# codeslake/RefVSR

Hardware: AMD Instinct MI355X
Metric: 4x SR frames/sec (270p->1080p, RefVSR_small_L1) (higher is better)
Workload: dtype f16; 1 GPU; config_RefVSR_small_L1 4x SR, 270x480 -> 1080x1920, frame_num=5, steady-state sliding window, n=1 (BASELINE configs[1]); synthetic clip seed 0, seeded random weights 1234; frames_per_rank=20, parallelism=frame-shard x1 (reset-aligned, no collective), window_cache=True, frame_ids=True, pipelined_calls=True, frames_per_call=4, headline_mode=frame groups, pipe_layout=pfm, full=False

## Files before the change

### include/refvsr_hip.h

```cpp
#ifndef REFVSR_HIP_H
#define REFVSR_HIP_H

#include <stddef.h>
#include <stdint.h>

#ifdef __cplusplus
extern "C" {
#endif

#define REFVSR_ABI_VERSION 15

int refvsr_abi_version(void);
int refvsr_max_maps(void);
const char* refvsr_last_error(void);
int refvsr_init(void);

int refvsr_num_cus(void);
int refvsr_stream_create_cu_range(int first_cu, int n_cus, void** stream);
int refvsr_stream_set_cu_budget(void* stream, int n_cus);
int refvsr_stream_destroy(void* stream);

enum { REFVSR_OUT_NHWC16 = 0, REFVSR_OUT_NHWC16_SHUFFLE2 = 1, REFVSR_OUT_PLANAR32 = 2 };

typedef struct RefvsrConv {
    const void* src0; int c0;
    const void* src1; int c1;
    int h_in, w_in;
    int h_out, w_out;
    int ksize, stride, pad;
    const void* wpack;
    const float* bias;
    int cout;
    int mt_per_block;
    int ksteps;
    float act_slope;
    const void* mul; int mul_c;
    const void* res; int res_c;
    float post_slope;
    int out_mode;
    void* out; int out_c;
    const float* res_planar;
    int f32;
    float add_const;
    float clamp_lo, clamp_hi;
    int batch; size_t bs_src0, bs_src1, bs_out, bs_res_planar;
} RefvsrConv;

int refvsr_conv_mfma(const RefvsrConv* d, void* stream);
int refvsr_set_conv_workgroup_cap(int cap);
int refvsr_conv_variant(const RefvsrConv* d, int* key);
int refvsr_kslot(int ty, int tx, int cg, int ksize, int ncg);
int refvsr_ksteps(int ksize, int ncg);

int refvsr_resblock_lean_fits(int c);
int refvsr_resblock_chain(const void* src, int c, int h, int w, int n, const void* const* w1, const float* const* b1,
                          const void* const* w2, const float* const* b2, int ksteps, float act_slope, float post_slope,
                          void* scratch0, void* scratch1, void* out, void* stream);
int refvsr_set_resblock_waves(int waves);
int refvsr_resblock_lean(const void* src, int c, int h, int w, const void* w1, const float* b1,
                         const void* w2, const float* b2, int ksteps, float act_slope, float post_slope,
                         void* out, void* stream);
#define REFVSR_RESBLOCK24_BLOB_BYTES 43264
int refvsr_resblock24_chain(const void* src, int h, int w, int n, const void* blobs, size_t blob_stride, float act_slope,
                            void* scratch0, void* scratch1, void* out, void* stream);
#define REFVSR_MAX_MAPS 4
int refvsr_resblock24_chain_batch(const void* const* src, int batch, int h, int w, int n, const void* blobs, size_t blob_stride,
                                  float act_slope, void* scratch0, void* scratch1, void* const* out, void* stream);
int refvsr_resblock24_kblock(int s, int q);
#define REFVSR_RESBLOCK24_F16W_BLOB_BYTES 28928
int refvsr_resblock24_f16w_blob_bytes(void);
int refvsr_resblock24_chain_f16w(const void* src, int h, int w, int n, const void* blobs, size_t blob_stride, float act_slope,
                                 void* scratch0, void* scratch1, void* out, void* stream);
int refvsr_resblock24_chain_batch_f16w(const void* const* src, int batch, int h, int w, int n, const void* blobs, size_t blob_stride,
                                       float act_slope, void* scratch0, void* scratch1, void* const* out, void* stream);
int refvsr_set_resblock24_waves(int waves);
#define REFVSR_RESBLOCK48_BLOB_BYTES 172544
int refvsr_resblock48_chain(const void* src, int h, int w, int n, const void* blobs, size_t blob_stride, float act_slope,
                            void* scratch0, void* scratch1, void* out, void* stream);
int refvsr_resblock48_chain_batch(const void* const* src, int batch, int h, int w, int n, const void* blobs, size_t blob_stride,
                                  float act_slope, void* scratch0, void* scratch1, void* const* out, void* stream);
int refvsr_set_resblock24_store(int mode);
int refvsr_conv24_supported(int c0, int c1);
int refvsr_conv24_blob_bytes(int c0, int c1);
int refvsr_conv24_kblock(int ncg, int s, int q);
int refvsr_conv24(const void* src0, int c0, const void* src1, int c1, int h, int w, const void* blob, float act_slope,
                  const void* mul, const void* res, float post_slope, void* out, void* stream);
int refvsr_conv24_batch(const void* const* src0, int c0, const void* const* src1, int c1, int batch, int h, int w, const void* blob,
                        float act_slope, const void* const* mul, const void* const* res, float post_slope, void* const* out,
                        void* stream);
int refvsr_conv_last_supported(int c);
int refvsr_conv_last_blob_bytes(int c);
int refvsr_conv_last(const void* src, int c, int h, int w, const void* blob, const float* base_lr, int bh, int bw,
                     float* out, void* stream);
int refvsr_conv_hr_last(const void* src, int h, int w, const void* blob, float act_slope, const float* base_lr, int bh, int bw,
                        float* out, void* stream);
enum { REFVSR_RESULT_F32 = 0, REFVSR_RESULT_F16 = 1, REFVSR_RESULT_U8 = 2 };
#define REFVSR_RESULT_FMT_MASK 0x0f
#define REFVSR_RESULT_HWC 0x10
int refvsr_convert_result_hwc(const float* src, int h, int w, int out_fmt, void* out, void* stream);
int refvsr_conv_last_fmt(const void* src, int c, int h, int w, const void* blob, const float* base_lr, int bh, int bw,
                         void* out, int out_fmt, void* stream);
int refvsr_conv_hr_last_fmt(const void* src, int h, int w, const void* blob, float act_slope, const float* base_lr, int bh, int bw,
                            void* out, int out_fmt, void* stream);
// ... 151 lines not shown
```

### refvsr_amd/csrc/conv_mfma.hip

```cpp
#include <type_traits>

#include "common.h"
#include "conv_plan.h"

struct ConvArgs {
    const unsigned char* src0; const unsigned char* src1;
    int c0, c1, ncg0, ncg, ps;
    int pixb0, pixb1;
    int h_in, w_in, h_out, w_out;
    int ks, stride, pad;
    int LH, LW;
    int G, S;
    float inv_ncg;
    const uint4* wpack; const float* bias;
    int cout;
    float act_slope, post_slope;
    const unsigned char* mul; int mul_c;
    const unsigned char* res; int res_c;
    int out_mode; void* out; int out_c;
    const float* res_planar; float add_const, clamp_lo, clamp_hi;
    int tab_bytes, wl_bytes;
    int gather;
    int tiles_x, n_xy;
    int prefetch;
    int grid;
    int ring;
    int batch;
    unsigned long long bs_src0, bs_src1, bs_out, bs_res_planar;
};

template <int MT, int TILES, bool F32, bool GATHER, bool RESIDENT, int EPI = 0, int NW = 4, bool HI1 = false>
__global__ __launch_bounds__(NW * 64) __attribute__((amdgpu_waves_per_eu(2, 4))) void conv_mfma_kernel(ConvArgs p) {
    constexpr int NT = NW * 64;
    static_assert(!(GATHER && RESIDENT), "gather mode streams its weights");
    static_assert(EPI == 0 || (RESIDENT && !F32), "the lean epilogue is built for the resident fp16 kernels");
    static_assert(!HI1 || (!F32 && !RESIDENT && !GATHER), "single-fp16 weights are built for the streamed fp16 kernels");
    constexpr int WFR = (F32 || HI1) ? 1 : 2;
    extern __shared__ __attribute__((aligned(16))) unsigned char smem[];
    int* tab = reinterpret_cast<int*>(smem);
    unsigned char* wl = smem + p.tab_bytes;
    unsigned char* tile = wl + p.wl_bytes;

    asm volatile("" :: "s"(p.src0), "s"(p.src1), "s"(p.wpack), "s"(p.bias), "s"(p.out), "s"(p.mul), "s"(p.res), "s"(p.c0),
                 "s"(p.ncg0), "s"(p.ncg), "s"(p.ps), "s"(p.pixb0), "s"(p.pixb1), "s"(p.h_in), "s"(p.w_in), "s"(p.h_out),
                 "s"(p.w_out), "s"(p.ks), "s"(p.stride), "s"(p.pad), "s"(p.LH), "s"(p.LW), "s"(p.G), "s"(p.S), "s"(p.inv_ncg),
                 "s"(p.cout), "s"(p.tab_bytes), "s"(p.wl_bytes), "s"(p.tiles_x), "s"(p.n_xy), "s"(p.grid));
    if (p.batch > 1) {
        const unsigned long long bi = blockIdx.y;
        p.src0 += bi * p.bs_src0;
        if (p.src1) p.src1 += bi * p.bs_src1;
        p.out = reinterpret_cast<unsigned char*>(p.out) + bi * p.bs_out;
        if (p.res_planar) p.res_planar = reinterpret_cast<const float*>(reinterpret_cast<const unsigned char*>(p.res_planar) + bi * p.bs_res_planar);
    }
    const int tid = threadIdx.x;
    const int lane = tid & 63;
    const int wave = tid >> 6;
    const int q = lane >> 4;
    const int lr = lane & 15;
    const int lp = (p.stride == 1) ? rv_pix16(lr) : lr;
    constexpr int TH = NW * TILES / 2;
    const int zg = blockIdx.z;

    for (int g = tid; g < p.S * 4; g += NT) {
        int off, slot;
        if (g < p.G) {
            const int tap = (int)(((float)g + 0.5f) * p.inv_ncg);
            const int cg = g - tap * p.ncg;
            const int ty = tap / p.ks;
            const int tx = tap - ty * p.ks;
            off = GATHER ? (ty | (tx << 8) | (cg << 16)) : ((ty * p.LW + tx) * p.ps + cg) * 16;
            slot = rv_kslot(ty, tx, cg, p.ks, p.ncg);
        } else {
            const int j = g - p.G;
            slot = rv_kpad_slot(j, p.ks, p.ncg);
            off = GATHER ? -1 : (slot < p.G ? 0 : (p.ncg > 1 ? 16 : (p.ks > 1 ? p.ps * 16 : 0)));
        }
        tab[slot] = off;
    }

    int pbase[TILES];
    if constexpr (!GATHER) {
#pragma unroll
        for (int t = 0; t < TILES; ++t) {
            const int ti = wave * TILES + t;
            pbase[t] = (((ti >> 1) * p.stride) * p.LW + ((ti & 1) * 16 + lp) * p.stride) * p.ps * 16;
// ... 288 lines not shown
                asm volatile("" : "+v"(e));
                if (e >= 0)
                    *reinterpret_cast<uint4*>(tile + (((e & 31) * p.LW + ((e >> 5) & 127)) * p.ps + ((e >> 20) & 127)) * 16) = xv[k];
            }
        };
        if (tl < k_hi) { x_fetch(tl); x_park(); }
        __syncthreads();
        for (; tl < k_hi; tl += k_step) {
            const bool has_next = tl + k_step < k_hi;
            if (has_next && p.prefetch) x_fetch(tl + k_step);
            asm volatile("" ::: "memory");
            zero_acc();
            compute_steps(wl, 0, p.S);
            __syncthreads();
            if (has_next) {
                if (!p.prefetch) x_fetch(tl + k_step);
                x_park();
            }
            asm volatile("" ::: "memory");
            int tide = tid;
            asm volatile("" : "+v"(tide));
            const int tyi = tl / p.tiles_x;
            if constexpr (EPI == 1) epilogue_lean(tyi * TH, (tl - tyi * p.tiles_x) * CONV_TW, tide);
            else epilogue(tyi * TH, (tl - tyi * p.tiles_x) * CONV_TW, tide);
            __syncthreads();
        }
    } else {
        const int tl = blockIdx.x;
        const int tyi = tl / p.tiles_x;
        const int tx0 = (tl - tyi * p.tiles_x) * CONV_TW;
        const int ty0 = tyi * TH;
        constexpr int PPW = GATHER ? 1 : CONV_CH * MT * WFR / NW;
        static_assert(GATHER || (PPW * NW == CONV_CH * MT * WFR && PPW >= 1 && 2 * PPW <= 60), "pieces per wave and chunk");
        constexpr int SLOT = CONV_CH * MT * WFR * 1024;
        const int NS = p.ring;
        const int wv = __builtin_amdgcn_readfirstlane(wave);
        const unsigned char* gw = reinterpret_cast<const unsigned char*>(wsrc) + lane * 16;
        auto issue = [&](const int c, const int slot) {
            const int np = min(CONV_CH, p.S - c * CONV_CH) * MT * WFR;
            const unsigned char* g = gw + (size_t)c * SLOT;
            unsigned char* l = wl + slot * SLOT;
#pragma unroll
            for (int j = 0; j < PPW; ++j) {
                const int pc = wv + j * NW;
                __builtin_amdgcn_global_load_lds((const __attribute__((address_space(1))) void*)(g + min(pc, np - 1) * 1024),
                                                 (__attribute__((address_space(3))) void*)(l + pc * 1024), 16, 0, 0);
            }
        };
        int slot_w = 0;
        if constexpr (!GATHER) {
            const int n_chunks = (p.S + CONV_CH - 1) / CONV_CH;
            for (int c = 0; c < min(NS - 1, n_chunks); ++c) { issue(c, slot_w); slot_w = slot_w + 1 == NS ? 0 : slot_w + 1; }
        }
        if constexpr (!GATHER) {
            const int iy0 = ty0 * p.stride - p.pad;
            const int ix0 = tx0 * p.stride - p.pad;
            const int row_chunks = p.LW * p.ncg;
            const float inv_rc = 1.0f / (float)row_chunks;
            const int total = p.LH * row_chunks;
            constexpr int SB = 8;
            for (int idx0 = tid; idx0 < total; idx0 += SB * NT) {
                uint4 sv[SB];
                int sd[SB];
#pragma unroll
                for (int k = 0; k < SB; ++k) {
                    const int idx = min(idx0 + k * NT, total - 1);
                    const int r = (int)(((float)idx + 0.5f) * inv_rc);
                    const int i = idx - r * row_chunks;
                    const int c = (int)(((float)i + 0.5f) * p.inv_ncg);
                    const int cg = i - c * p.ncg;
                    const int iy = iy0 + r;
                    const int ix = ix0 + c;
                    const bool ok = (unsigned)iy < (unsigned)p.h_in && (unsigned)ix < (unsigned)p.w_in;
                    const size_t pix = (size_t)min(max(iy, 0), p.h_in - 1) * p.w_in + min(max(ix, 0), p.w_in - 1);
                    const unsigned char* g = (cg < p.ncg0) ? p.src0 + pix * p.pixb0 + cg * 16 : p.src1 + pix * p.pixb1 + (cg - p.ncg0) * 16;
                    uint4 v = *reinterpret_cast<const uint4*>(g);
                    const unsigned keep = ok ? 0xffffffffu : 0u;
                    v.x &= keep; v.y &= keep; v.z &= keep; v.w &= keep;
                    sv[k] = v;
                    sd[k] = ((r * p.LW + c) * p.ps + cg) * 16;
                }
#pragma unroll
                for (int k = 0; k < SB; ++k)
                    if (idx0 + k * NT < total) *reinterpret_cast<uint4*>(tile + sd[k]) = sv[k];
            }
        } else {
#pragma unroll
            for (int t = 0; t < TILES; ++t) {
                const int ti = wave * TILES + t;
                const int iy = (ty0 + (ti >> 1)) * p.stride - p.pad + 4096, ix = (tx0 + (ti & 1) * 16 + lp) * p.stride - p.pad + 4096;
                pbase[t] = (iy << 16) | ix;
            }
        }
        if constexpr (!GATHER) {
            const unsigned lds_tab = (unsigned)(size_t)(__attribute__((address_space(3))) unsigned char*)reinterpret_cast<unsigned char*>(tab);
            const unsigned lds_wl = (unsigned)(size_t)(__attribute__((address_space(3))) unsigned char*)wl;
            const unsigned lds_tile = (unsigned)(size_t)(__attribute__((address_space(3))) unsigned char*)tile;
            unsigned pbaddr[TILES];
#pragma unroll
            for (int t = 0; t < TILES; ++t) pbaddr[t] = lds_tile + (unsigned)pbase[t];
            typedef unsigned u32x4 __attribute__((ext_vector_type(4)));
            auto ld128 = [](const unsigned addr) {
                u32x4 v;
                asm volatile("ds_read_b128 %0, %1" : "=v"(v) : "v"(addr));
                return make_uint4(v[0], v[1], v[2], v[3]);
            };
            auto tie = [](uint4& r) {
                u32x4 t = {r.x, r.y, r.z, r.w};
                asm volatile("" : "+v"(t));
                r = make_uint4(t[0], t[1], t[2], t[3]);
            };
            auto wait_set = [&](uint4 (&a)[NA], uint4 (&b)[TILES]) {
                asm volatile("s_waitcnt lgkmcnt(%0)" :: "n"(NA + TILES) : "memory");
#pragma unroll
                for (int i = 0; i < NA; ++i) tie(a[i]);
#pragma unroll
                for (int t = 0; t < TILES; ++t) tie(b[t]);
            };
            static_assert(NA + TILES <= 15, "lgkmcnt range");
            auto compute_chunk = [&](const unsigned wslot, const int s0, const int ns) {
                unsigned toff[CONV_CH];
#pragma unroll
                for (int j = 0; j < CONV_CH; ++j)
                    asm volatile("ds_read_b32 %0, %1" : "=v"(toff[j]) : "v"(lds_tab + (unsigned)(((s0 + min(j, ns - 1)) * 4 + q) * 4)));
                asm volatile("s_waitcnt lgkmcnt(0)" ::: "memory");
#pragma unroll
                for (int j = 0; j < CONV_CH; ++j) asm volatile("" : "+v"(toff[j]));
                const unsigned wa = wslot + (unsigned)lane * 16;
                auto load_set = [&](auto jc, uint4 (&a)[NA], uint4 (&b)[TILES]) {
                    constexpr int j = decltype(jc)::value;
                    const unsigned wj = wa + (unsigned)min(j, ns - 1) * (NA * 1024);
#pragma unroll
                    for (int i = 0; i < NA; ++i) {
                        u32x4 v;
                        asm volatile("ds_read_b128 %0, %1 offset:%2" : "=v"(v) : "v"(wj), "n"(i * 1024));
                        a[i] = make_uint4(v[0], v[1], v[2], v[3]);
                    }
#pragma unroll
                    for (int t = 0; t < TILES; ++t) b[t] = ld128(pbaddr[t] + toff[j]);
                };
                uint4 a0[NA], b0[TILES], a1[NA], b1[TILES];
                load_set(std::integral_constant<int, 0>{}, a0, b0);
#define RV_RING_PAIR(J)                                                                     \
                load_set(std::integral_constant<int, (J) + 1>{}, a1, b1);                   \
                wait_set(a0, b0);                                                           \
                __builtin_amdgcn_sched_barrier(0);                                          \
                if ((J) < ns) mfma_step(a0, b0);                                            \
                load_set(std::integral_constant<int, (J) + 2>{}, a0, b0);                   \
                wait_set(a1, b1);                                                           \
                __builtin_amdgcn_sched_barrier(0);                                          \
                if ((J) + 1 < ns) mfma_step(a1, b1);
                RV_RING_PAIR(0) RV_RING_PAIR(2) RV_RING_PAIR(4)
#undef RV_RING_PAIR
                static_assert(CONV_CH == 8, "the ring loop is unrolled for 8 K-steps per chunk");
                load_set(std::integral_constant<int, 7>{}, a1, b1);
                wait_set(a0, b0);
                __builtin_amdgcn_sched_barrier(0);
                if (6 < ns) mfma_step(a0, b0);
                asm volatile("s_waitcnt lgkmcnt(0)" ::: "memory");
#pragma unroll
                for (int i = 0; i < NA; ++i) tie(a1[i]);
#pragma unroll
                for (int t = 0; t < TILES; ++t) tie(b1[t]);
                __builtin_amdgcn_sched_barrier(0);
                if (7 < ns) mfma_step(a1, b1);
            };
            const int n_chunks = (p.S + CONV_CH - 1) / CONV_CH;
            zero_acc();
            int slot_r = 0;
            for (int c = 0; c < n_chunks; ++c) {
                const int after = min(NS - 2, n_chunks - 1 - c);
                if (after <= 0) asm volatile("s_waitcnt vmcnt(0)" ::: "memory");
                else if (after == 1) asm volatile("s_waitcnt vmcnt(%0)" :: "n"(PPW) : "memory");
                else asm volatile("s_waitcnt vmcnt(%0)" :: "n"(2 * PPW) : "memory");
                asm volatile("s_waitcnt lgkmcnt(0)" ::: "memory");
                __builtin_amdgcn_s_barrier();
                asm volatile("" ::: "memory");
                if (c + NS - 1 < n_chunks) { issue(c + NS - 1, slot_w); slot_w = slot_w + 1 == NS ? 0 : slot_w + 1; }
                compute_chunk(lds_wl + (unsigned)slot_r * SLOT, c * CONV_CH, min(CONV_CH, p.S - c * CONV_CH));
                slot_r = slot_r + 1 == NS ? 0 : slot_r + 1;
            }
        } else {
            constexpr int WPT = (CONV_CH * MT * WFR * 64) / NT;
            const int n_chunks = (p.S + CONV_CH - 1) / CONV_CH;
            static_assert(WPT <= 12, "prefetch register set");
            uint4 w0, w1, w2, w3, w4, w5, w6, w7, w8, w9, w10, w11;
    #define RV_W_ALL(OP) OP(0) OP(1) OP(2) OP(3) OP(4) OP(5) OP(6) OP(7) OP(8) OP(9) OP(10) OP(11)
    #define RV_W_LOAD(k) if constexpr (WPT > k) w##k = g[min(tid + k * NT, n16n - 1)];
    #define RV_W_STORE(k) if constexpr (WPT > k) { if (tid + k * NT < n16n) d[tid + k * NT] = w##k; }
            {
                const int n16 = min(CONV_CH, p.S) * MT * WFR * 64;
                uint4* d = reinterpret_cast<uint4*>(wl);
                for (int i = tid; i < n16; i += NT) d[i] = wsrc[i];
            }
            zero_acc();
            __syncthreads();
            for (int c = 0; c < n_chunks; ++c) {
                const int s0 = c * CONV_CH;
                const int ns = min(CONV_CH, p.S - s0);
                const bool has_next = (c + 1 < n_chunks);
                const int sn = has_next ? s0 + CONV_CH : s0;
                const int n16n = min(CONV_CH, p.S - sn) * MT * WFR * 64;
                {
                    const uint4* g = wsrc + (size_t)sn * MT * WFR * 64;
                    RV_W_ALL(RV_W_LOAD)
                }
                compute_steps(wl, s0, ns);
                if (has_next) {
                    __syncthreads();
                    uint4* d = reinterpret_cast<uint4*>(wl);
                    RV_W_ALL(RV_W_STORE)
                    __syncthreads();
                }
            }
        }
        epilogue(ty0, tx0, tid);
    }
}

static int g_wg_cap = 0;
extern "C" int refvsr_set_conv_workgroup_cap(int cap) {
    g_wg_cap = cap > 0 ? cap : 0;
    return 0;
}

extern "C" int refvsr_kslot(int ty, int tx, int cg, int ksize, int ncg) { return rv_kslot(ty, tx, cg, ksize, ncg); }
extern "C" int refvsr_ksteps(int ksize, int ncg) { return rv_ksteps(ksize, ncg); }

template <int MT, int TILES, bool F32, bool GATHER, bool RESIDENT, int EPI, int NW, bool HI1>
static int launch_conv(ConvArgs& a, int nz, size_t lds, hipStream_t st) {
    static RvLaunchCap lc = {};
    int gx = a.n_xy, cap = 0;
    if (int rc = rv_launch_cap(lc, &conv_mfma_kernel<MT, TILES, F32, GATHER, RESIDENT, EPI, NW, HI1>, NW * 64, 160 * 1024, lds, st,
                               RESIDENT ? &cap : nullptr, nz * a.batch))
        return rc;
    if (RESIDENT) {
        if (g_wg_cap > 0) cap = g_wg_cap;
        if (gx > cap) gx = cap;
    }
    a.grid = gx;
    hipLaunchKernelGGL((conv_mfma_kernel<MT, TILES, F32, GATHER, RESIDENT, EPI, NW, HI1>), dim3(gx, a.batch, nz), dim3(NW * 64), lds, st, a);
    RV_LAUNCH_CHECK();
    return 0;
}

static ConvArgs conv_args(const RefvsrConv* d, const ConvPlan& p) {
    const int cgrp = p.F32 ? 4 : 8, esz = p.F32 ? 4 : 2;
    ConvArgs a;
    memset(&a, 0, sizeof(a));
    a.src0 = (const unsigned char*)d->src0; a.src1 = (const unsigned char*)d->src1;
    a.c0 = d->c0; a.c1 = d->c1;
    a.pixb0 = d->c0 * esz; a.pixb1 = d->c1 * esz;
    a.ncg0 = d->c0 / cgrp; a.ncg = (d->c0 + d->c1) / cgrp;
    a.ps = p.ps;
    a.h_in = d->h_in; a.w_in = d->w_in; a.h_out = d->h_out; a.w_out = d->w_out;
    a.ks = d->ksize; a.stride = d->stride; a.pad = d->pad;
    a.LH = p.LH; a.LW = p.LW;
    a.G = p.G; a.S = p.S;
    a.inv_ncg = 1.0f / (float)a.ncg;
    a.wpack = (const uint4*)d->wpack; a.bias = d->bias; a.cout = d->cout;
    a.act_slope = d->act_slope; a.post_slope = d->post_slope;
    a.mul = (const unsigned char*)d->mul; a.mul_c = d->mul_c;
    a.res = (const unsigned char*)d->res; a.res_c = d->res_c;
    a.out_mode = d->out_mode; a.out = d->out; a.out_c = d->out_c;
    a.res_planar = d->res_planar; a.add_const = d->add_const;
    a.clamp_lo = d->clamp_lo; a.clamp_hi = d->clamp_hi;
    a.tab_bytes = p.tab_bytes; a.wl_bytes = p.wl_bytes;
    a.gather = p.gather; a.ring = p.ring; a.prefetch = p.prefetch;
    a.tiles_x = p.tiles_x; a.n_xy = p.n_xy;
    a.batch = d->batch > 1 ? d->batch : 1;
    if (a.batch > 1) { a.bs_src0 = d->bs_src0; a.bs_src1 = d->bs_src1; a.bs_out = d->bs_out; a.bs_res_planar = d->bs_res_planar; }
    return a;
}

static const ConvKnobs& conv_knobs() {
    static const ConvKnobs knobs = conv_knobs_from_env();
    return knobs;
}

extern "C" int refvsr_conv_variant(const RefvsrConv* d, int* key) {
    RV_CHECK(key != nullptr, "conv_variant: null key");
    ConvPlan p;
    if (int rc = conv_plan(d, conv_knobs(), &p)) return rc;
    *key = p.key();
    return 0;
}

extern "C" int refvsr_conv_mfma(const RefvsrConv* d, void* stream) {
    ConvPlan p;
    if (int rc = conv_plan(d, conv_knobs(), &p)) return rc;
    RV_CHECK(refvsr_init() == 0, "init failed");
    ConvArgs a = conv_args(d, p);
    switch (p.key()) {
#define RV_CONV_CASE(...) case conv_variant_key(__VA_ARGS__): return launch_conv<__VA_ARGS__>(a, p.nz, p.lds, (hipStream_t)stream);
        RV_CONV_VARIANTS(RV_CONV_CASE)
#undef RV_CONV_CASE
    }
    refvsr_set_error("conv: no kernel for MT=%d tiles=%d", p.MT, p.TILES);
    return 1;
}
```

### refvsr_amd/csrc/conv_plan.h

```cpp
#pragma once
#include <stddef.h>
#include <stdlib.h>

#include "../../include/refvsr_hip.h"
#include "plan_common.h"

#define CONV_CH 8
#define CONV_RES_MAX 16
#define CONV_XPF 8
#define CONV_TW 32

#define RV_CONV_VARIANTS(X)                                                                                          \
                                                                          \
    X(1, 4, false, true, false, 0, 4, false) X(2, 4, false, true, false, 0, 4, false) X(3, 4, false, true, false, 0, 4, false) \
                                                       \
    X(1, 2, false, false, false, 0, 8, true) X(2, 2, false, false, false, 0, 8, true)                                \
    X(1, 4, false, false, false, 0, 4, true) X(2, 4, false, false, false, 0, 4, true)                                \
    X(1, 2, false, false, false, 0, 4, true) X(2, 2, false, false, false, 0, 4, true)                                \
                                                                               \
    X(3, 2, false, false, true, 1, 16, false) X(3, 2, false, false, true, 0, 16, false)                              \
    X(2, 2, false, false, true, 1, 16, false) X(2, 2, false, false, true, 0, 16, false)                              \
                                                               \
    X(1, 2, false, false, true, 1, 8, false) X(1, 2, false, false, true, 0, 8, false) X(1, 2, false, false, false, 0, 8, false) \
    X(2, 2, false, false, true, 1, 8, false) X(2, 2, false, false, true, 0, 8, false) X(2, 2, false, false, false, 0, 8, false) \
    X(3, 2, false, false, true, 1, 8, false) X(3, 2, false, false, true, 0, 8, false) X(3, 2, false, false, false, 0, 8, false) \
                                                                                     \
    X(1, 1, true, false, true, 0, 8, false) X(1, 1, true, false, false, 0, 8, false)                                 \
    X(2, 1, true, false, true, 0, 8, false) X(2, 1, true, false, false, 0, 8, false)                                 \
               \
    RV_CONV_VARIANTS4(X, 1, 2) RV_CONV_VARIANTS4(X, 1, 4) RV_CONV_VARIANTS4(X, 2, 2) RV_CONV_VARIANTS4(X, 2, 4)     \
    RV_CONV_VARIANTS4(X, 3, 2) RV_CONV_VARIANTS4(X, 3, 4)
#define RV_CONV_VARIANTS4(X, M, T)                                                                                   \
    X(M, T, true, false, true, 0, 4, false) X(M, T, true, false, false, 0, 4, false)                                 \
    X(M, T, false, false, true, 1, 4, false) X(M, T, false, false, true, 0, 4, false) X(M, T, false, false, false, 0, 4, false)

constexpr int conv_variant_key(int MT, int TILES, bool F32, bool GATHER, bool RESIDENT, int EPI, int NW, bool HI1) {
    return MT | TILES << 2 | NW << 6 | EPI << 11 | (int)F32 << 12 | (int)GATHER << 13 | (int)RESIDENT << 14 | (int)HI1 << 15;
}

struct ConvKnobs {
    bool no_persist = false;
    int res_max = CONV_RES_MAX;
    int tiles = 0;
    bool no_w16 = false;
    int ring = 0;
    bool no_nw8 = false;
    bool no_prefetch = false;
    bool no_lean_epi = false;
};
static inline ConvKnobs conv_knobs_from_env() {
    ConvKnobs k;
    auto num = [](const char* name, int dflt) { const char* v = getenv(name); return v ? atoi(v) : dflt; };
    k.no_persist = getenv("REFVSR_CONV_NO_PERSIST") != nullptr;
    k.res_max = num("REFVSR_CONV_RES_MAX", CONV_RES_MAX);
    k.tiles = num("REFVSR_CONV_TILES", 0);
    k.no_w16 = getenv("REFVSR_CONV_NO_W16") != nullptr;
    k.ring = num("REFVSR_CONV_RING", 0);
    k.no_nw8 = getenv("REFVSR_CONV_NO_NW8") != nullptr;
    k.no_prefetch = getenv("REFVSR_CONV_NO_PREFETCH") != nullptr;
    k.no_lean_epi = getenv("REFVSR_CONV_NO_LEAN_EPI") != nullptr;
    return k;
}

struct ConvPlan {
    int MT, TILES; bool F32, GATHER, RESIDENT; int EPI, NW; bool HI1;
    int nz;
    size_t lds;
    int tab_bytes, wl_bytes;
    int ring;
    int LH, LW;
    int ps;
    int G, S;
    int tiles_x, n_xy;
    int gather;
    int prefetch;
    int key() const { return conv_variant_key(MT, TILES, F32, GATHER, RESIDENT, EPI, NW, HI1); }
};

static int conv_plan(const RefvsrConv* d, const ConvKnobs& knobs, ConvPlan* p) {
    RV_CHECK(d != nullptr, "conv: null descriptor");
    *p = ConvPlan();
    const bool f32 = d->f32 == 1;
    const bool hi1 = d->f32 == 2;
    RV_CHECK(d->f32 >= 0 && d->f32 <= 2, "conv: weight mode (f32) must be 0, 1 or 2");
    const int cgrp = f32 ? 4 : 8;
    RV_CHECK(d->src0 && d->c0 > 0 && d->c0 % cgrp == 0, "conv: src0/c0 invalid (c0=%d)", d->c0);
    RV_CHECK((d->src1 == nullptr) == (d->c1 == 0) && d->c1 % cgrp == 0, "conv: src1/c1 invalid (c1=%d)", d->c1);
    RV_CHECK(d->ksize >= 1 && d->ksize <= 7 && d->stride >= 1 && d->pad >= 0, "conv: bad geometry");
    RV_CHECK(d->h_in > 0 && d->w_in > 0 && d->h_out > 0 && d->w_out > 0, "conv: bad sizes");
    RV_CHECK(d->wpack && d->bias && d->out, "conv: null weights/bias/out");
    RV_CHECK(d->mt_per_block >= 1 && d->mt_per_block <= 3, "conv: mt_per_block must be 1..3");
    RV_CHECK(d->cout >= 1, "conv: cout");
    if (d->out_mode != REFVSR_OUT_PLANAR32) {
        RV_CHECK(d->cout % 4 == 0 && d->out_c % 4 == 0, "conv: nhwc16 output needs cout %% 4 == 0");
        RV_CHECK(d->res_planar == nullptr, "conv: res_planar only with planar output");
    }
    if (d->out_mode == REFVSR_OUT_NHWC16_SHUFFLE2)
        RV_CHECK(d->cout % 16 == 0 && !d->mul && !d->res && !f32 && d->out_c >= d->cout / 4 && d->out_c - d->cout / 4 <= 4,
                 "conv: pixel-shuffle output constraints");
    const int ncg = (d->c0 + d->c1) / cgrp, ks = d->ksize, stride = d->stride;
    p->ps = ncg | 1;
    p->G = ks * ks * ncg;
    p->S = rv_ksteps(ks, ncg);
    RV_CHECK(p->S == d->ksteps, "conv: ksteps mismatch (descriptor %d, geometry %d)", d->ksteps, p->S);
    RV_CHECK(d->batch >= 0 && d->batch <= 65535, "conv: batch out of range (%d)", d->batch);
    if (d->batch > 1) {
        RV_CHECK(!d->mul && !d->res, "conv: batch > 1 takes no mul / res operands");
        RV_CHECK(d->bs_src0 % 16 == 0 && d->bs_src1 % 16 == 0 && d->bs_out % 8 == 0 && d->bs_res_planar % 4 == 0, "conv: batch strides must keep the maps aligned");
        RV_CHECK(d->bs_src0 > 0 && d->bs_out > 0 && (!d->src1 || d->bs_src1 > 0) && (!d->res_planar || d->bs_res_planar > 0), "conv: batch strides missing");
    }

    const int MT = d->mt_per_block, S = p->S;
    p->nz = rv_cdiv(rv_cdiv(d->cout, 16), MT);
    p->tab_bytes = ((S * 4 * 4 + 15) / 16) * 16;
    const int wfr_kb = MT * ((f32 || hi1) ? 1 : 2) * 1024;
    const size_t LDS_MAX = 160 * 1024;

    int tiles = 4;
    size_t lds = 0;
    auto tile_bytes = [&](int tl) {
        p->LH = (tl * 2 - 1) * stride + ks;
        p->LW = (CONV_TW - 1) * stride + ks;
        return (size_t)p->LH * p->LW * p->ps * 16;
    };
    bool resident = false, one_wg = false;
    bool w16 = false;
    if (!knobs.no_persist && !hi1 && S <= knobs.res_max && S <= CONV_RES_MAX) {
        int best_wg = 0;
        for (int tl = 4; tl >= 2; tl -= 2) {
            if (knobs.tiles && tl != knobs.tiles) continue;
            const size_t tb = tile_bytes(tl);
            const size_t need = (size_t)p->tab_bytes + (size_t)S * wfr_kb + tb;
// ... 76 lines not shown
```

### refvsr_amd/hip.py

```python
import ctypes as C
import os

_HERE = os.path.dirname(os.path.abspath(__file__))
LIB_PATH = os.path.join(_HERE, 'librefvsr_hip.so')

OUT_NHWC16, OUT_NHWC16_SHUFFLE2, OUT_PLANAR32 = 0, 1, 2
RS_BICUBIC, RS_BILINEAR, RS_BILINEAR_AC, RS_NEAREST = 0, 1, 2, 3
RESULT_F32, RESULT_F16, RESULT_U8 = 0, 1, 2
RESULT_HWC = 0x10
INGEST_PLANAR, INGEST_HWC = 0, 1
MATCH_KP, MATCH_ROWCHUNK, MATCH_COLBLOCK = 152, 256, 512
ABI_VERSION = 15
MAX_MAPS = 4
INGEST_MAX_FRAMES = 16
SCORE_MAX_FRAMES = 16
SCORE_MAX_RECTS = 8
COLORMAP_MAX_MAPS = 16
FINGERPRINT_CHUNK_WORDS = 4096
RESBLOCK24_BLOB_BYTES = 43264
RESBLOCK24_F16W_BLOB_BYTES = 28928
RESBLOCK48_BLOB_BYTES = 172544


class RefvsrConv(C.Structure):
    _fields_ = [
        ('src0', C.c_void_p), ('c0', C.c_int),
        ('src1', C.c_void_p), ('c1', C.c_int),
        ('h_in', C.c_int), ('w_in', C.c_int),
        ('h_out', C.c_int), ('w_out', C.c_int),
        ('ksize', C.c_int), ('stride', C.c_int), ('pad', C.c_int),
        ('wpack', C.c_void_p), ('bias', C.c_void_p),
        ('cout', C.c_int), ('mt_per_block', C.c_int), ('ksteps', C.c_int),
        ('act_slope', C.c_float),
        ('mul', C.c_void_p), ('mul_c', C.c_int),
        ('res', C.c_void_p), ('res_c', C.c_int),
        ('post_slope', C.c_float),
        ('out_mode', C.c_int),
        ('out', C.c_void_p), ('out_c', C.c_int),
        ('res_planar', C.c_void_p),
        ('f32', C.c_int),
        ('add_const', C.c_float), ('clamp_lo', C.c_float), ('clamp_hi', C.c_float),
        ('batch', C.c_int), ('bs_src0', C.c_size_t), ('bs_src1', C.c_size_t), ('bs_out', C.c_size_t), ('bs_res_planar', C.c_size_t),
    ]


_P, _I, _F, _Z = C.c_void_p, C.c_int, C.c_float, C.c_size_t

SIGNATURES = {
    'refvsr_init': [],
    'refvsr_max_maps': [],
    'refvsr_num_cus': [],
    'refvsr_stream_create_cu_range': [_I, _I, C.POINTER(C.c_void_p)],
    'refvsr_stream_set_cu_budget': [_P, _I],
    'refvsr_stream_destroy': [_P],
    'refvsr_conv_mfma': [C.POINTER(RefvsrConv), _P],
    'refvsr_set_conv_workgroup_cap': [_I],
    'refvsr_conv_variant': [C.POINTER(RefvsrConv), C.POINTER(C.c_int)],
    'refvsr_kslot': [_I, _I, _I, _I, _I],
    'refvsr_ksteps': [_I, _I],
    'refvsr_set_probe': [_P, _I],
    'refvsr_resblock_lean_fits': [_I],
    'refvsr_set_resblock_waves': [_I],
    'refvsr_resblock_lean': [_P, _I, _I, _I, _P, _P, _P, _P, _I, _F, _F, _P, _P],
    'refvsr_resblock_chain': [_P, _I, _I, _I, _I, _P, _P, _P, _P, _I, _F, _F, _P, _P, _P, _P],
    'refvsr_resblock24_chain': [_P, _I, _I, _I, _P, _Z, _F, _P, _P, _P, _P],
    'refvsr_resblock48_chain': [_P, _I, _I, _I, _P, _Z, _F, _P, _P, _P, _P],
    'refvsr_resblock24_kblock': [_I, _I],
    'refvsr_set_resblock24_waves': [_I],
    'refvsr_set_resblock24_store': [_I],
    'refvsr_conv24_supported': [_I, _I],
    'refvsr_conv24_blob_bytes': [_I, _I],
    'refvsr_conv24_kblock': [_I, _I, _I],
    'refvsr_conv24': [_P, _I, _P, _I, _I, _I, _P, _F, _P, _P, _F, _P, _P],
    'refvsr_conv32_supported': [_I, _I],
    'refvsr_conv32_blob_bytes': [_I, _I],
    'refvsr_conv32': [_P, _I, _P, _I, _I, _I, _P, _F, _P, _P, _F, _P, _P],
    'refvsr_conv48_supported': [_I, _I],
    'refvsr_conv48_blob_bytes': [_I, _I],
    'refvsr_conv48': [_P, _I, _P, _I, _I, _I, _P, _F, _P, _P, _F, _P, _P],
    'refvsr_conv_shuffle2_supported': [_I],
    'refvsr_conv_shuffle2_blob_bytes': [_I],
    'refvsr_conv_shuffle2': [_P, _I, _I, _I, _P, _F, _P, _P],
    'refvsr_conv_direct_f32': [_P, _I, _I, _I, _P, _P, _I, _I, _I, _I, _F, _P, _I, _I, _P],
    'refvsr_conv1x1_f32': [_P, _I, _I, _I, _P, _P, _F, _P, _P],
    'refvsr_pack_nhwc16': [_P, _I, _I, _I, _P, _I, _P],
    'refvsr_pack_nhwc32': [_P, _I, _I, _I, _P, _I, _P],
    'refvsr_unpack_nhwc16': [_P, _I, _I, _I, _I, _P, _P],
    'refvsr_resize': [_P, _I, _I, _I, _P, _I, _I, _I, _F, _F, _P, _P, _P, _I, _I, _I, _P],
    'refvsr_avgpool2': [_P, _I, _I, _I, _P, _P],
    'refvsr_maxpool2': [_P, _I, _I, _I, _P, _P],
    'refvsr_max2': [_P, _P, _P, _Z, _P],
    'refvsr_buffers_equal': [_P, _P, _I, _Z, _P, _P],
    'refvsr_warp_nhwc16': [_P, _I, _I, _I, _P, _I, _I, _P, _P],
    'refvsr_warp_nhwc16_up2': [_P, _I, _I, _I, _P, _I, _I, _P, _P],
    'refvsr_warp_planar': [_P, _I, _I, _I, _P, _I, _I, _P, _P],
    'refvsr_spynet_level_input': [_P, _P, _P, _I, _I, _P, _P, _P],
    'refvsr_conv_hr_last': [_P, _I, _I, _P, _F, _P, _I, _I, _P, _P],
    'refvsr_conv_last_supported': [_I],
    'refvsr_conv_last_blob_bytes': [_I],
    'refvsr_conv_last': [_P, _I, _I, _I, _P, _P, _I, _I, _P, _P],
    'refvsr_conv_last_fmt': [_P, _I, _I, _I, _P, _P, _I, _I, _P, _I, _P],
    'refvsr_conv_hr_last_fmt': [_P, _I, _I, _P, _F, _P, _I, _I, _P, _I, _P],
    'refvsr_convert_result': [_P, _Z, _I, _P, _P],
    'refvsr_convert_result_hwc': [_P, _I, _I, _I, _P, _P],
    'refvsr_conf_alpha': [_P, _P, _I, _I, _I, _P, _P, _F, _P, _I, _F, _P, _P, _P],
    'refvsr_spynet_level_input_batch': [_P, _P, _I, _P, _I, _I, _P, _P, _P],
    'refvsr_resblock24_chain_batch': [_P, _I, _I, _I, _I, _P, _Z, _F, _P, _P, _P, _P],
    'refvsr_resblock48_chain_batch': [_P, _I, _I, _I, _I, _P, _Z, _F, _P, _P, _P, _P],
    'refvsr_conv24_batch': [_P, _I, _P, _I, _I, _I, _I, _P, _F, _P, _P, _F, _P, _P],
# ... 84 lines not shown
```

### refvsr_amd/ops.py

```python
import ctypes as C
import math
import os

import numpy as np
import torch

from . import fingerprint, hip
from .knobs import env_flag
from .packing import BlobFlags, blob_plan, pack_conv24, pack_conv_shuffle2, pack_resblock
from .hip import (OUT_NHWC16, OUT_NHWC16_SHUFFLE2, OUT_PLANAR32, RS_BICUBIC, RS_BILINEAR,
                  RS_BILINEAR_AC, RS_NEAREST)


_STREAM = None


def _stream():
    if _STREAM is not None:
        return _STREAM
    return C.c_void_p(torch.cuda.current_stream().cuda_stream)


class on_stream(object):

# ... 847 lines not shown

def warp_nhwc16_up2(x, flow_lr):
    _nhwc(x)
    _planar(flow_lr, 2)
    hin, win, cs = x.shape
    hl, wl = flow_lr.shape[1:]
    out = torch.empty((2 * hl, 2 * wl, cs), dtype=torch.float16, device=x.device)
    hip.check(hip.lib().refvsr_warp_nhwc16_up2(_ptr(x), hin, win, cs, _ptr(flow_lr), hl, wl, _ptr(out), _stream()), 'warp_nhwc16_up2')
    return out


def warp_planar(x, flow):
    _planar(x)
    _planar(flow, 2)
    c, hin, win = x.shape
    hf, wf = flow.shape[1:]
    out = torch.empty((c, hf, wf), dtype=torch.float32, device=x.device)
    hip.check(hip.lib().refvsr_warp_planar(_ptr(x), c, hin, win, _ptr(flow), hf, wf, _ptr(out), _stream()), 'warp_planar')
    return out


def spynet_level_input(ref, supp, flow_prev):
    _planar(ref, 3)
    _planar(supp, 3)
    h, w = ref.shape[1:]
    if flow_prev is not None:
        _planar(flow_prev, 2)
        assert tuple(flow_prev.shape[1:]) == (h // 2, w // 2)
    out8 = torch.empty((h, w, 8), dtype=torch.float16, device=ref.device)
    fup = torch.empty((2, h, w), dtype=torch.float32, device=ref.device)
    hip.check(hip.lib().refvsr_spynet_level_input(_ptr(ref), _ptr(supp), _ptr(flow_prev), h, w, _ptr(out8), _ptr(fup),
                                                  _stream()), 'spynet_level_input')
    return out8, fup


def spynet_level_input_batch(refs, supps, flow_prev):
    B = len(refs)
    assert 1 <= B <= 8 and len(supps) == B
    for t_ in list(refs) + list(supps):
        _planar(t_, 3)
    h, w = refs[0].shape[1:]
    if flow_prev is not None:
        assert flow_prev.is_cuda and flow_prev.dtype == torch.float32 and flow_prev.is_contiguous() and \
            tuple(flow_prev.shape) == (B, 2, h // 2, w // 2)
    out8 = torch.empty((B, h, w, 8), dtype=torch.float16, device=refs[0].device)
    fup = torch.empty((B, 2, h, w), dtype=torch.float32, device=refs[0].device)
    pr = (C.c_void_p * B)(*[t_.data_ptr() for t_ in refs])
    ps = (C.c_void_p * B)(*[t_.data_ptr() for t_ in supps])
    hip.check(hip.lib().refvsr_spynet_level_input_batch(pr, ps, B, _ptr(flow_prev), h, w, _ptr(out8), _ptr(fup), _stream()),
              'spynet_level_input_batch')
    return out8, fup


def set_match_patches_kernel(mode):
    hip.check(hip.lib().refvsr_set_match_patches_kernel(int(mode)), 'set_match_patches_kernel')


def match_patches(feat, row_pad, want_lo=False):
    _planar(feat, 16)
    h, w = feat.shape[1:]
    n = h * w
    rows = torch.empty((_round_up(n, row_pad), hip.MATCH_KP), dtype=torch.float16, device=feat.device)
    inv = torch.empty((n,), dtype=torch.float32, device=feat.device)
    lo = torch.empty_like(rows) if want_lo else None
    if rows.shape[0] > n:
        rows[n:].zero_()
        if lo is not None:
            lo[n:].zero_()
    hip.check(hip.lib().refvsr_match_patches(_ptr(feat), h, w, _ptr(rows), _ptr(inv), _ptr(lo), _stream()), 'match_patches')
    return (rows, inv, lo) if want_lo else (rows, inv)


def match_top2(ref_rows, n_ref, lr_rows, n_lr, row_splits=1):
    assert ref_rows.shape[0] % hip.MATCH_ROWCHUNK == 0 and lr_rows.shape[0] % hip.MATCH_COLBLOCK == 0
    assert ref_rows.shape[0] >= n_ref and lr_rows.shape[0] >= n_lr
    ci = torch.empty((n_lr, 2 * row_splits), dtype=torch.int32, device=ref_rows.device)
    cv = torch.empty((n_lr, 2 * row_splits), dtype=torch.float32, device=ref_rows.device)
    hip.check(hip.lib().refvsr_match_top2(_ptr(ref_rows), n_ref, _ptr(lr_rows), n_lr, row_splits, _ptr(ci), _ptr(cv),
                                          _stream()), 'match_top2')
    return ci, cv


MATCH_EXACT_MARGIN = 2.5e-4


def match_refine(lr_feat, ref_feat, inv_lr, inv_ref, cand, cand_val=None, margin=None, lr_split=None, ref_split=None):
    _planar(lr_feat, 16)
    _planar(ref_feat, 16)
    h, w = lr_feat.shape[1:]
    hr, wr = ref_feat.shape[1:]
    assert cand.dtype == torch.int32 and cand.shape[0] == h * w and cand.is_contiguous()
    conf = torch.empty((h * w,), dtype=torch.float32, device=lr_feat.device)
    idx = torch.empty((h * w,), dtype=torch.int32, device=lr_feat.device)
    if margin is None:
        hip.check(hip.lib().refvsr_match_refine(_ptr(lr_feat), h, w, _ptr(ref_feat), hr, wr, _ptr(inv_lr), _ptr(inv_ref),
                                                _ptr(cand), None, cand.shape[1], 0.0, None, _ptr(conf), _ptr(idx), _stream()),
                  'match_refine')
        return conf, idx
    assert cand_val is not None and ref_split is not None and lr_split is not None
    assert cand_val.shape == cand.shape and cand_val.is_contiguous()
    (lr_rows, lr_lo), (ref_rows, ref_lo) = lr_split, ref_split
    sparse_lo = lr_lo is None
    if sparse_lo:
        lr_lo = torch.empty_like(lr_rows)
    for r, n_, pad in ((lr_rows, h * w, 1), (lr_lo, h * w, 1), (ref_rows, hr * wr, hip.MATCH_ROWCHUNK), (ref_lo, hr * wr, hip.MATCH_ROWCHUNK)):
        assert r.dtype == torch.float16 and r.is_contiguous() and r.shape[1] == hip.MATCH_KP
# ... 209 lines not shown
```

Measured before the change: 241.7 frames/s.

## Make streamed conv kernels persistent with next-tile input prefetch in registers

Adds a persistent 'walk' mode for streamed-weight MFMA conv kernels. The grid is capped to the resident workgroup count, and each workgroup loops over several output tiles. While the weight ring K-loop runs on the current tile, the next tile's input halo is prefetched into registers, then parked into LDS after a barrier. By default this applies only to plans with large LDS footprints (over 80KB), and one HI1 NW8 variant gets a higher minimum waves-per-EU hint. The aim is to hide input-tile load latency and launch tail, at the cost of heavier register pressure and more complex vmcnt accounting.

```diff
diff --git a/include/refvsr_hip.h b/include/refvsr_hip.h
--- a/include/refvsr_hip.h
+++ b/include/refvsr_hip.h
@@ -48,7 +48,9 @@
 
 int refvsr_conv_mfma(const RefvsrConv* d, void* stream);
 int refvsr_set_conv_workgroup_cap(int cap);
+int refvsr_set_conv_stream_walk(int on);
 int refvsr_conv_variant(const RefvsrConv* d, int* key);
+int refvsr_conv_stream_walk(const RefvsrConv* d, int* walk);
 int refvsr_kslot(int ty, int tx, int cg, int ksize, int ncg);
 int refvsr_ksteps(int ksize, int ncg);
 
diff --git a/refvsr_amd/csrc/conv_mfma.hip b/refvsr_amd/csrc/conv_mfma.hip
--- a/refvsr_amd/csrc/conv_mfma.hip
+++ b/refvsr_amd/csrc/conv_mfma.hip
@@ -25,12 +25,13 @@
     int prefetch;
     int grid;
     int ring;
+    int walk;
     int batch;
     unsigned long long bs_src0, bs_src1, bs_out, bs_res_planar;
 };
 
 template <int MT, int TILES, bool F32, bool GATHER, bool RESIDENT, int EPI = 0, int NW = 4, bool HI1 = false>
-__global__ __launch_bounds__(NW * 64) __attribute__((amdgpu_waves_per_eu(2, 4))) void conv_mfma_kernel(ConvArgs p) {
+__global__ __launch_bounds__(NW * 64) __attribute__((amdgpu_waves_per_eu(conv_min_waves(GATHER, RESIDENT, NW, HI1), 4))) void conv_mfma_kernel(ConvArgs p) {
     constexpr int NT = NW * 64;
     static_assert(!(GATHER && RESIDENT), "gather mode streams its weights");
     static_assert(EPI == 0 || (RESIDENT && !F32), "the lean epilogue is built for the resident fp16 kernels");
@@ -425,7 +426,9 @@
             const int n_chunks = (p.S + CONV_CH - 1) / CONV_CH;
             for (int c = 0; c < min(NS - 1, n_chunks); ++c) { issue(c, slot_w); slot_w = slot_w + 1 == NS ? 0 : slot_w + 1; }
         }
-        if constexpr (!GATHER) {
+        constexpr int SXPF = GATHER ? 0 : conv_stream_xpf(MT, TILES, F32, NW, HI1);
+        const bool walking = SXPF > 0 && p.walk != 0;
+        if constexpr (!GATHER) { if (!walking) {
             const int iy0 = ty0 * p.stride - p.pad;
             const int ix0 = tx0 * p.stride - p.pad;
             const int row_chunks = p.LW * p.ncg;
@@ -457,7 +460,7 @@
                 for (int k = 0; k < SB; ++k)
                     if (idx0 + k * NT < total) *reinterpret_cast<uint4*>(tile + sd[k]) = sv[k];
             }
-        } else {
+        } } else {
 #pragma unroll
             for (int t = 0; t < TILES; ++t) {
                 const int ti = wave * TILES + t;
@@ -539,20 +542,116 @@
                 if (7 < ns) mfma_step(a1, b1);
             };
             const int n_chunks = (p.S + CONV_CH - 1) / CONV_CH;
+            int slot_r = 0;
+            static_assert(2 * PPW + SXPF <= 63, "vmcnt range");
+            auto ring_k_loop = [&](const bool pf) {
+                for (int c = 0; c < n_chunks; ++c) {
+                    const int after = min(NS - 2, n_chunks - 1 - c);
+                    if (SXPF > 0 && pf && c < NS - 1) {
+                        if (after <= 0) asm volatile("s_waitcnt vmcnt(%0)" :: "n"(SXPF) : "memory");
+                        else if (after == 1) asm volatile("s_waitcnt vmcnt(%0)" :: "n"(PPW + SXPF) : "memory");
+                        else asm volatile("s_waitcnt vmcnt(%0)" :: "n"(2 * PPW + SXPF) : "memory");
+                    } else if (after <= 0) asm volatile("s_waitcnt vmcnt(0)" ::: "memory");
+                    else if (after == 1) asm volatile("s_waitcnt vmcnt(%0)" :: "n"(PPW) : "memory");
+                    else asm volatile("s_waitcnt vmcnt(%0)" :: "n"(2 * PPW) : "memory");
+                    asm volatile("s_waitcnt lgkmcnt(0)" ::: "memory");
+                    __builtin_amdgcn_s_barrier();
+                    asm volatile("" ::: "memory");
+                    if (c + NS - 1 < n_chunks) { issue(c + NS - 1, slot_w); slot_w = slot_w + 1 == NS ? 0 : slot_w + 1; }
+                    compute_chunk(lds_wl + (unsigned)slot_r * SLOT, c * CONV_CH, min(CONV_CH, p.S - c * CONV_CH));
+                    slot_r = slot_r + 1 == NS ? 0 : slot_r + 1;
+                }
+            };
+            if constexpr (SXPF > 0) {
+            if (walking) {
+                int tl, k_hi;
+                rv_tile_range(p.n_xy, p.grid, tl, k_hi);
+                const int row_chunks = p.LW * p.ncg;
+                const int total = p.LH * row_chunks;
+                unsigned xq[(SXPF + 1) / 2];
+                {
+                    const float inv_rc = 1.0f / (float)row_chunks;
+#pragma unroll
+                    for (int k = 0; k < SXPF; ++k) {
+                        const int idx = min(tid + k * NT, total - 1);
+                        const int r = (int)(((float)idx + 0.5f) * inv_rc);
+                        const int i = idx - r * row_chunks;
+                        const int c = (int)(((float)i + 0.5f) * p.inv_ncg);
+                        const int cg = i - c * p.ncg;
+                        const unsigned e = (unsigned)(r | (c << 5) | (cg << 12));
+                        if (k & 1) xq[k >> 1] |= e << 16;
+                        else xq[k >> 1] = e;
+                    }
+                }
+                uint4 xv[SXPF];
+                auto x_desc = [&](const int k) {
+                    unsigned w = xq[k >> 1];
+                    asm volatile("" : "+v"(w));
+                    return (k & 1) ? w >> 16 : w & 0xffffu;
+                };
+                auto x_fetch = [&](const int t) {
+                    const int tyi = t / p.tiles_x;
+                    const int iy0 = tyi * TH * p.stride - p.pad;
+                    const int ix0 = (t - tyi * p.tiles_x) * CONV_TW * p.stride - p.pad;
+#pragma unroll
+                    for (int k = 0; k < SXPF; ++k) {
+                        const unsigned e = x_desc(k);
+                        const int iy = iy0 + (int)(e & 31), ix = ix0 + (int)((e >> 5) & 127), cg = (int)(e >> 12);
+                        const size_t pix = (size_t)min(max(iy, 0), p.h_in - 1) * p.w_in + min(max(ix, 0), p.w_in - 1);
+                        const unsigned char* g = cg >= p.ncg0 ? p.src1 + pix * p.pixb1 + (cg - p.ncg0) * 16 : p.src0 + pix * p.pixb0 + cg * 16;
+                        xv[k] = *reinterpret_cast<const uint4*>(g);
+                        __builtin_amdgcn_sched_barrier(0);
+                    }
+                };
+                auto x_park = [&](const int t) {
+                    const int tyi = t / p.tiles_x;
+                    const int iy0 = tyi * TH * p.stride - p.pad;
+                    const int ix0 = (t - tyi * p.tiles_x) * CONV_TW * p.stride - p.pad;
+#pragma unroll
+                    for (int k = 0; k < SXPF; ++k) {
+                        const unsigned e = x_desc(k);
+                        const int r = (int)(e & 31), c = (int)((e >> 5) & 127), cg = (int)(e >> 12);
+                        const bool ok = (unsigned)(iy0 + r) < (unsigned)p.h_in && (unsigned)(ix0 + c) < (unsigned)p.w_in;
+                        const unsigned keep = ok ? 0xffffffffu : 0u;
+                        uint4 v = xv[k];
+                        v.x &= keep; v.y &= keep; v.z &= keep; v.w &= keep;
+                        *reinterpret_cast<uint4*>(tile + ((r * p.LW + c) * p.ps + cg) * 16) = v;
+                        __builtin_amdgcn_sched_barrier(0);
+                    }
+                };
+                x_fetch(tl);
+                x_park(tl);
+#pragma unroll
+                for (int m = 0; m < MT; ++m)
+                    asm volatile("" :: "v"(bias_r[m].x), "v"(bias_r[m].y), "v"(bias_r[m].z), "v"(bias_r[m].w));
+                for (; tl < k_hi; ++tl) {
+                    const bool has_next = tl + 1 < k_hi;
+                    asm volatile("" ::: "memory");
+                    if (has_next) x_fetch(tl + 1);
+                    asm volatile("" ::: "memory");
+                    zero_acc();
+                    ring_k_loop(has_next);
+                    asm volatile("" ::: "memory");
+                    __builtin_amdgcn_s_barrier();
+                    asm volatile("" ::: "memory");
+#pragma unroll
+                    for (int k = 0; k < SXPF; ++k) asm volatile("" :: "v"(xv[k].x));
+                    if (has_next) {
+                        x_park(tl + 1);
+                        asm volatile("" ::: "memory");
+                        for (int c = 0; c < min(NS - 1, n_chunks); ++c) { issue(c, slot_w); slot_w = slot_w + 1 == NS ? 0 : slot_w + 1; }
+                    }
+                    asm volatile("" ::: "memory");
+                    int tide = tid;
+                    asm volatile("" : "+v"(tide));
+                    const int tyi = tl / p.tiles_x;
+                    epilogue(tyi * TH, (tl - tyi * p.tiles_x) * CONV_TW, tide);
+                }
+                return;
+            }
+            }
             zero_acc();
-            int slot_r = 0;
-            for (int c = 0; c < n_chunks; ++c) {
-                const int after = min(NS - 2, n_chunks - 1 - c);
-                if (after <= 0) asm volatile("s_waitcnt vmcnt(0)" ::: "memory");
-                else if (after == 1) asm volatile("s_waitcnt vmcnt(%0)" :: "n"(PPW) : "memory");
-                else asm volatile("s_waitcnt vmcnt(%0)" :: "n"(2 * PPW) : "memory");
-                asm volatile("s_waitcnt lgkmcnt(0)" ::: "memory");
-                __builtin_amdgcn_s_barrier();
-                asm volatile("" ::: "memory");
-                if (c + NS - 1 < n_chunks) { issue(c + NS - 1, slot_w); slot_w = slot_w + 1 == NS ? 0 : slot_w + 1; }
-                compute_chunk(lds_wl + (unsigned)slot_r * SLOT, c * CONV_CH, min(CONV_CH, p.S - c * CONV_CH));
-                slot_r = slot_r + 1 == NS ? 0 : slot_r + 1;
-            }
+            ring_k_loop(false);
         } else {
             constexpr int WPT = (CONV_CH * MT * WFR * 64) / NT;
             const int n_chunks = (p.S + CONV_CH - 1) / CONV_CH;
@@ -596,6 +695,12 @@
     g_wg_cap = cap > 0 ? cap : 0;
     return 0;
 }
+static int g_stream_walk = 1;
+extern "C" int refvsr_set_conv_stream_walk(int on) {
+    g_stream_walk = on <= 0 ? 0 : on >= 2 ? 2 : 1;
+    return 0;
+}
+static int conv_walks(const ConvPlan& p) { return g_stream_walk == 2 ? p.walk_fits : (g_stream_walk ? p.walk : 0); }
 
 extern "C" int refvsr_kslot(int ty, int tx, int cg, int ksize, int ncg) { return rv_kslot(ty, tx, cg, ksize, ncg); }
 extern "C" int refvsr_ksteps(int ksize, int ncg) { return rv_ksteps(ksize, ncg); }
@@ -604,14 +709,16 @@
 static int launch_conv(ConvArgs& a, int nz, size_t lds, hipStream_t st) {
     static RvLaunchCap lc = {};
     int gx = a.n_xy, cap = 0;
+    const bool walk = !RESIDENT && a.walk;
     if (int rc = rv_launch_cap(lc, &conv_mfma_kernel<MT, TILES, F32, GATHER, RESIDENT, EPI, NW, HI1>, NW * 64, 160 * 1024, lds, st,
-                               RESIDENT ? &cap : nullptr, nz * a.batch))
+                               RESIDENT || walk ? &cap : nullptr, nz * a.batch))
         return rc;
-    if (RESIDENT) {
+    if (RESIDENT || walk) {
         if (g_wg_cap > 0) cap = g_wg_cap;
         if (gx > cap) gx = cap;
     }
     a.grid = gx;
+    a.walk = walk && gx < a.n_xy;
     hipLaunchKernelGGL((conv_mfma_kernel<MT, TILES, F32, GATHER, RESIDENT, EPI, NW, HI1>), dim3(gx, a.batch, nz), dim3(NW * 64), lds, st, a);
     RV_LAUNCH_CHECK();
     return 0;
@@ -639,7 +746,7 @@
     a.res_planar = d->res_planar; a.add_const = d->add_const;
     a.clamp_lo = d->clamp_lo; a.clamp_hi = d->clamp_hi;
     a.tab_bytes = p.tab_bytes; a.wl_bytes = p.wl_bytes;
-    a.gather = p.gather; a.ring = p.ring; a.prefetch = p.prefetch;
+    a.gather = p.gather; a.ring = p.ring; a.prefetch = p.prefetch; a.walk = p.walk;
     a.tiles_x = p.tiles_x; a.n_xy = p.n_xy;
     a.batch = d->batch > 1 ? d->batch : 1;
     if (a.batch > 1) { a.bs_src0 = d->bs_src0; a.bs_src1 = d->bs_src1; a.bs_out = d->bs_out; a.bs_res_planar = d->bs_res_planar; }
@@ -659,11 +766,20 @@
     return 0;
 }
 
+extern "C" int refvsr_conv_stream_walk(const RefvsrConv* d, int* walk) {
+    RV_CHECK(walk != nullptr, "conv_stream_walk: null result");
+    ConvPlan p;
+    if (int rc = conv_plan(d, conv_knobs(), &p)) return rc;
+    *walk = conv_walks(p);
+    return 0;
+}
+
 extern "C" int refvsr_conv_mfma(const RefvsrConv* d, void* stream) {
     ConvPlan p;
     if (int rc = conv_plan(d, conv_knobs(), &p)) return rc;
     RV_CHECK(refvsr_init() == 0, "init failed");
     ConvArgs a = conv_args(d, p);
+    a.walk = conv_walks(p);
     switch (p.key()) {
 #define RV_CONV_CASE(...) case conv_variant_key(__VA_ARGS__): return launch_conv<__VA_ARGS__>(a, p.nz, p.lds, (hipStream_t)stream);
         RV_CONV_VARIANTS(RV_CONV_CASE)
diff --git a/refvsr_amd/csrc/conv_plan.h b/refvsr_amd/csrc/conv_plan.h
--- a/refvsr_amd/csrc/conv_plan.h
+++ b/refvsr_amd/csrc/conv_plan.h
@@ -9,6 +9,11 @@
 #define CONV_RES_MAX 16
 #define CONV_XPF 8
 #define CONV_TW 32
+
+constexpr int conv_stream_xpf(int MT, int TILES, bool F32, int NW, bool HI1) {
+    return (HI1 && NW == 8 && TILES == 2) ? 9 : (F32 && NW == 4 && TILES == 4 && MT == 2) ? 22 : (!F32 && !HI1 && NW == 4 && TILES == 2 && MT == 1) ? 24 : 0;
+}
+constexpr int conv_min_waves(bool GATHER, bool RESIDENT, int NW, bool HI1) { return (!GATHER && !RESIDENT && HI1 && NW == 8) ? 4 : 2; }
 
 #define RV_CONV_VARIANTS(X)                                                                                          \
                                                                           \
@@ -47,6 +52,8 @@
     bool no_nw8 = false;
     bool no_prefetch = false;
     bool no_lean_epi = false;
+    bool no_stream_walk = false;
+    bool stream_walk_all = false;
 };
 static inline ConvKnobs conv_knobs_from_env() {
     ConvKnobs k;
@@ -59,6 +66,8 @@
     k.no_nw8 = getenv("REFVSR_CONV_NO_NW8") != nullptr;
     k.no_prefetch = getenv("REFVSR_CONV_NO_PREFETCH") != nullptr;
     k.no_lean_epi = getenv("REFVSR_CONV_NO_LEAN_EPI") != nullptr;
+    k.no_stream_walk = getenv("REFVSR_CONV_NO_STREAM_WALK") != nullptr;
+    k.stream_walk_all = getenv("REFVSR_CONV_STREAM_WALK_ALL") != nullptr;
     return k;
 }
 
@@ -74,10 +83,22 @@
     int tiles_x, n_xy;
     int gather;
     int prefetch;
+    int walk;
+    int walk_fits;
     int key() const { return conv_variant_key(MT, TILES, F32, GATHER, RESIDENT, EPI, NW, HI1); }
 };
 
+static int conv_plan_variant(const RefvsrConv* d, const ConvKnobs& knobs, ConvPlan* p);
 static int conv_plan(const RefvsrConv* d, const ConvKnobs& knobs, ConvPlan* p) {
+    if (int rc = conv_plan_variant(d, knobs, p)) return rc;
+    const int xpf = conv_stream_xpf(p->MT, p->TILES, p->F32, p->NW, p->HI1);
+    const int ncg = (d->c0 + d->c1) / (p->F32 ? 4 : 8);
+    p->walk_fits = !knobs.no_stream_walk && !p->RESIDENT && !p->GATHER && xpf > 0 && p->LH * p->LW * ncg <= xpf * p->NW * 64 && p->LH <= 31 &&
+                   p->LW <= 127 && ncg <= 16 && p->n_xy < (1 << 20);
+    p->walk = p->walk_fits && (knobs.stream_walk_all || p->lds > 80 * 1024);
+    return 0;
+}
+static int conv_plan_variant(const RefvsrConv* d, const ConvKnobs& knobs, ConvPlan* p) {
     RV_CHECK(d != nullptr, "conv: null descriptor");
     *p = ConvPlan();
     const bool f32 = d->f32 == 1;
diff --git a/refvsr_amd/hip.py b/refvsr_amd/hip.py
--- a/refvsr_amd/hip.py
+++ b/refvsr_amd/hip.py
@@ -55,6 +55,8 @@
     'refvsr_stream_destroy': [_P],
     'refvsr_conv_mfma': [C.POINTER(RefvsrConv), _P],
     'refvsr_set_conv_workgroup_cap': [_I],
+    'refvsr_set_conv_stream_walk': [_I],
+    'refvsr_conv_stream_walk': [C.POINTER(RefvsrConv), C.POINTER(C.c_int)],
     'refvsr_conv_variant': [C.POINTER(RefvsrConv), C.POINTER(C.c_int)],
     'refvsr_kslot': [_I, _I, _I, _I, _I],
     'refvsr_ksteps': [_I, _I],
diff --git a/refvsr_amd/ops.py b/refvsr_amd/ops.py
--- a/refvsr_amd/ops.py
+++ b/refvsr_amd/ops.py
@@ -923,6 +923,10 @@
     return out8, fup
 
 
+def set_conv_stream_walk(on):
+    hip.check(hip.lib().refvsr_set_conv_stream_walk(int(on)), 'set_conv_stream_walk')
+
+
 def set_match_patches_kernel(mode):
     hip.check(hip.lib().refvsr_set_match_patches_kernel(int(mode)), 'set_match_patches_kernel')
 
```

Result: no change. 242.0 frames/s (median of 3 runs) (+0.1%).
